# ilyakurdyukov/jpeg-quantsmooth

Measured on AMD Instinct MI355X. Metric: 8x8 blocks/s at q=3 niter=3, higher is better.
Workload: dtype f32

## Files before the change

### include/jpegqs_hip.h

```cpp
#ifndef JPEGQS_HIP_H
#define JPEGQS_HIP_H

#include <stddef.h>
#include <stdint.h>

#ifdef __cplusplus
extern "C" {
#endif

#define QS_HIP_MAXC 4

enum {
	QS_HIP_OK = 0,
	QS_HIP_ENODEV = -1,
	QS_HIP_EINVAL = -2,
	QS_HIP_ENOMEM = -3,
	QS_HIP_ENOTSUP = -4
};


typedef struct {
	int32_t ncomp;
	int32_t colorspace;
	int32_t image_width, image_height;
// ... 234 lines not shown
const char *qs_hip_last_error(void);
#define QS_HIP_ABI_VERSION 7
int qs_hip_abi_version(void);

size_t qs_hip_consts_bytes(void);
size_t qs_hip_plane_pitch(int wblk);
size_t qs_hip_plane_bytes(int wblk, int hblk);
size_t qs_hip_plane_row_offset(int wblk, int y);

int qs_hip_consts_build(void *host_out, const uint16_t quant[64], int flags);

int qs_hip_idct_plane(const void *d_consts, int16_t *d_coef, uint8_t *d_plane,
		int wblk, int hblk, int first, int rep_top, int rep_bot,
		int32_t *d_status, void *stream);

int qs_hip_smooth_plane(const void *d_consts, int16_t *d_coef, const uint8_t *d_plane,
		int wblk, int hblk, int flags, int luma, int final_clamp, void *stream);
int qs_hip_smooth_plane_next(const void *d_consts, int16_t *d_coef, const uint8_t *d_plane, uint8_t *d_plane_next,
		int wblk, int hblk, int flags, int luma, int final_clamp, int rep_top, int rep_bot, void *stream);
int qs_hip_smooth_rows(const void *d_consts, int16_t *d_coef, const uint8_t *d_plane,
		int wblk, int hblk, int row0, int row1, int flags, int luma, int final_clamp, void *stream);

#define QS_HIP_MAX_PLANES 56
typedef struct {
	const void *d_consts;
	int16_t *d_coef;
	uint8_t *d_plane;
	int32_t *d_status;
	int32_t wblk, hblk, luma;
	int32_t band;
} qs_hip_plane_ref;
#define QS_HIP_PLANE_DEFER 4
#define QS_HIP_FIRST_DEFER 2
int qs_hip_idct_planes(const qs_hip_plane_ref *refs, int n, int first, void *stream);
int qs_hip_smooth_planes(const qs_hip_plane_ref *refs, int n, int flags, int final_clamp, void *stream);
int qs_hip_smooth_planes_next(const qs_hip_plane_ref *refs, uint8_t *const *d_plane_next, int n, int flags,
		int final_clamp, void *stream);

int qs_hip_joint_plane(const void *d_consts, int16_t *d_coef, const uint8_t *d_plane,
		const uint8_t *d_luma_lowres, int wblk, int hblk,
		int rebalance, int final_clamp, void *stream);
int qs_hip_lowq_plane(const void *d_consts, int16_t *d_coef, const uint8_t *d_plane,
		int wblk, int hblk, int rebalance, int final_clamp, void *stream);
int qs_hip_downsample_plane(const uint8_t *d_luma, int ywblk, int yhblk, uint8_t *d_lowres,
		int lwblk, int lhblk, int ws, int hs, void *stream);
size_t qs_hip_upsample_pitch(int image_width, int ws);
size_t qs_hip_upsample_bytes(int image_width, int image_height, int ws, int hs);
int qs_hip_upsample_plane(const uint8_t *d_chroma, const uint8_t *d_luma_lowres, int cwblk,
		const uint8_t *d_luma, int ywblk, int yhblk, uint8_t *d_pixels,
		int image_width, int image_height, int ws, int hs, void *stream);
int qs_hip_upsample_rows(const uint8_t *d_chroma, const uint8_t *d_luma_lowres, int cwblk,
		const uint8_t *d_luma, int ywblk, int yhblk, uint8_t *d_pixels, size_t pitch,
		int w1, int h1, int first_rows, int ws, int hs, void *stream);
int qs_hip_fdct_plane(const uint8_t *d_pixels, size_t pitch, int16_t *d_coef, int wblk, int hblk, void *stream);

int qs_hip_clamp_plane(int16_t *d_coef, int wblk, int hblk, void *stream);
int qs_hip_dequant_plane(const void *d_consts, int16_t *d_coef, int wblk, int hblk, void *stream);

#ifdef __cplusplus
}
#endif
#endif
```

### jpeg-quantsmooth_amd/bands.py

```python
from __future__ import annotations

import os
from dataclasses import dataclass


_LIB = None


def _lib():
    global _LIB
    if _LIB is None:
        try:
            from .hipqs import HipQS
            _LIB = HipQS()
        except (OSError, RuntimeError, ImportError):
            _LIB = False
    return _LIB or None


def _band_rows_py(hblk: int, world: int, rank: int, align: int = 1):
    if hblk < 0 or world < 1 or not 0 <= rank < world or align < 1:
        raise ValueError("band_rows: bad argument")
    units = (hblk + align - 1) // align
    a, b = units * rank // world * align, units * (rank + 1) // world * align
# ... 148 lines not shown
        o = offs[y]
        return planes2d[:, o:o + pitch]
    ops, recvs = [], []
    for nbr, src_y, dst_y in ((topo.up, 0, -1), (topo.down, h - 1, h)):
        if nbr is None:
            continue
        out = view(src_y).contiguous()
        if hostcopy:
            out = out.to("cpu")
        buf = out.new_empty(out.shape)
        ops.append(dist.P2POp(dist.isend, out, nbr))
        ops.append(dist.P2POp(dist.irecv, buf, nbr))
        recvs.append((dst_y, buf))
    if ops:
        for w in dist.batch_isend_irecv(ops):
            w.wait()
    for dst_y, buf in recvs:
        view(dst_y).copy_(buf)


def run_bands_batched(engines, topo: BandTopology, niter: int, exchange_many) -> None:
    for it in range(niter):
        for e in engines:
            e.idct(it == 0, topo.rep_top, topo.rep_bot)
        exchange_many()
        for e in engines:
            e.smooth(it == niter - 1)


def defer_bit() -> int:
    return 0 if os.environ.get("QS_BANDS_DEFER", "1") == "0" else 4


def run_bands_batched_sets(hip, engines, topo: BandTopology, niter: int, exchange_many, stream=None, mark=None, fused=True) -> None:
    band = (1 if topo.up is not None else 0) | (2 if topo.down is not None else 0)
    flags = engines[0].flags
    s = stream if stream is not None else engines[0]._s()
    if fused:
        for e in engines:
            e.ensure_plane2()
    for it in range(niter):
        q = defer_bit() if it == 0 else 0
        if it == 0 or not fused:
            refs = hip.plane_refs([(e.cst.data_ptr(), e.coef.data_ptr(), e.plane.data_ptr(), e.status.data_ptr(),
                                    e.wblk, e.hblk, e.luma, band | q) for e in engines])
            hip.idct_planes(refs, it == 0, s)
        exchange_many()
        nxt = fused and it < niter - 1
        refs = hip.plane_refs([(e.cst.data_ptr(), e.coef.data_ptr(), e.plane.data_ptr(), e.status.data_ptr(),
                                e.wblk, e.hblk, e.luma, band | q, e.plane2.data_ptr() if nxt else None) for e in engines])
        if mark:
            mark(0)
        hip.smooth_planes(refs, flags, it == niter - 1, s)
        if mark:
            mark(1)
        if nxt:
            for e in engines:
                e.plane, e.plane2 = e.plane2, e.plane


def run_band_edge_first(hip, e, topo: BandTopology, niter: int, exchange, main, side, torch) -> None:
    if e.hblk < 3:
        return run_bands_batched_sets(hip, [e], topo, niter, exchange, stream=main.cuda_stream)
    e.ensure_plane2()
    band_top = 1 if topo.up is not None else 0
    band_bot = 2 if topo.down is not None else 0
    pitch, wb, hb = e.pitch, e.wblk, e.hblk
    row_bytes = wb * 128

    def views(cur, nxt, q):
        c0, p0 = e.coef.data_ptr(), cur.data_ptr()
        n0 = nxt.data_ptr() if nxt is not None else None
        at = lambda base, r: base + r * 8 * pitch if base is not None else None
        top = (e.cst.data_ptr(), c0, p0, e.status.data_ptr(), wb, 1, e.luma, band_top | 2 | q, n0)
        bot = (e.cst.data_ptr(), c0 + (hb - 1) * row_bytes, at(p0, hb - 1), e.status.data_ptr(), wb, 1, e.luma, 1 | band_bot | q, at(n0, hb - 1))
        mid = (e.cst.data_ptr(), c0 + row_bytes, at(p0, 1), e.status.data_ptr(), wb, hb - 2, e.luma, 3 | q, at(n0, 1))
        return hip.plane_refs([top, bot]), hip.plane_refs([mid])
    ev_main, ev_edge = torch.cuda.Event(), torch.cuda.Event()
    whole = hip.plane_refs([(e.cst.data_ptr(), e.coef.data_ptr(), e.plane.data_ptr(), e.status.data_ptr(), wb, hb, e.luma,
                             band_top | band_bot | (defer_bit() if niter > 0 else 0))])
    hip.idct_planes(whole, True, main.cuda_stream)
    ev_main.record(main)
    side.wait_event(ev_main)
# ... 399 lines not shown
```

### jpeg-quantsmooth_amd/csrc/check_kernel_budget.py

```python
#!/usr/bin/env python3
import re
import sys

KERNELS = ("qs_smooth_plane_kernel", "qs_smooth_set_kernel")
MAX_VGPRS = 168
MAX_LDS = 160 * 1024 // 3
FIELDS = ("group_segment_fixed_size", "private_segment_fixed_size", "vgpr_count")


def kernel_records(text):
    m = re.search(r"^\s*\.amdgpu_metadata\s*$(.*?)^\s*\.end_amdgpu_metadata\s*$", text, re.S | re.M)
    if not m:
        return {}
    recs, cur = [], None
    for line in m.group(1).split("\n"):
        if re.match(r"  - \.", line):
            cur = {}
            recs.append(cur)
            line = "    " + line[4:]
        f = re.match(r"    \.(\w+):\s*(\S+)\s*$", line)
        if f and cur is not None:
            cur[f.group(1)] = f.group(2)
    return {r["name"]: {k: int(r[k]) for k in FIELDS if k in r} for r in recs if "name" in r}


def main(path):
    recs = {n: r for n, r in kernel_records(open(path).read()).items() if any(k in n for k in KERNELS)}
    if len(recs) != 4 or any(len(r) != len(FIELDS) for r in recs.values()):
        print(f"check_kernel_budget: ERROR: expected the metadata of 4 recovery kernels in {path}, found {sorted(recs)}", file=sys.stderr)
        return 1
    bad = 0
    for n, r in sorted(recs.items()):
        why = []
        if r["private_segment_fixed_size"] != 0:
            why.append(f"{r['private_segment_fixed_size']} B of scratch per lane (spills)")
        if r["vgpr_count"] > MAX_VGPRS:
            why.append(f"{r['vgpr_count']} VGPRs > {MAX_VGPRS} (three waves per SIMD)")
        if r["group_segment_fixed_size"] > MAX_LDS:
            why.append(f"{r['group_segment_fixed_size']} B of LDS > {MAX_LDS} (three workgroups per CU)")
        print(f"check_kernel_budget: {n}: {r['vgpr_count']} VGPRs, {r['private_segment_fixed_size']} B scratch, "
              f"{r['group_segment_fixed_size']} B LDS" + (" -- ERROR: " + "; ".join(why) if why else ""),
              file=sys.stderr if why else sys.stdout)
        bad += bool(why)
    return 1 if bad else 0


SPLIT_READ_KERNELS = ("qrs_map", "qrs_decode", "qrs_count", "qrs_tile_scan", "qrs_write", "qrs_dc_tiles", "qrs_dc_write")
DECODE_KERNELS = ("qs_decode_kernel", "qs_decode_scaled_kernel")
PROG_KERNELS = ("qp_begin", "qp_nofile", "qp_flags", "qp_headscan", "qp_runs", "qp_size", "qp_emit", "qp_frame",
                "qr_flags", "qr_wsum", "qr_wscan", "qr_next", "qr_hop")
READ_PROG_KERNELS = ("qrp_init", "qrp_check", "qrp_decode")
INSTANCES = {"qp_size": 4, "qp_emit": 2}


def main_no_scratch(prefix, path):
    want = [k for k in SPLIT_READ_KERNELS + DECODE_KERNELS + PROG_KERNELS + READ_PROG_KERNELS if k.startswith(prefix)]
    recs = kernel_records(open(path).read())
    bad = 0
    for k in want:
        hits = {n: r for n, r in recs.items() if re.search(rf"\d+{k}[EI\d]", n)}
        if len(hits) != INSTANCES.get(k, 1) or any("private_segment_fixed_size" not in r for r in hits.values()):
            count = {1: "one kernel"}.get(INSTANCES.get(k, 1), f"{INSTANCES.get(k, 1)} kernels")
            print(f"check_kernel_budget: ERROR: expected the metadata of {count} {k} in {path}, found {sorted(hits)}", file=sys.stderr)
            bad += 1
            continue
        for n, r in sorted(hits.items()):
            scratch = r["private_segment_fixed_size"]
            print(f"check_kernel_budget: {n}: {r.get('vgpr_count')} VGPRs, {scratch} B scratch, {r.get('group_segment_fixed_size')} B LDS"
                  + (" -- ERROR: scratch" if scratch else ""), file=sys.stderr if scratch else sys.stdout)
            bad += bool(scratch)
    return 1 if bad or not want else 0


if __name__ == "__main__":
    if len(sys.argv) == 4 and sys.argv[1] == "--no-scratch":
        sys.exit(main_no_scratch(sys.argv[2], sys.argv[3]))
    sys.exit(main(sys.argv[1]))
```

### jpeg-quantsmooth_amd/csrc/qs_device.h

```cpp
#pragma once
#include <stdint.h>

#define QS_APRON_X 16
#define QS_LDS_PITCH 65
#define QS_TAB_MAX 272

enum {
  QS_DIAGONALS = 1, QS_JOINT_YUV = 2, QS_UPSAMPLE_UV = 4, QS_LOW_QUALITY = 8,
  QS_NO_REBALANCE = 16, QS_NO_REBALANCE_UV = 32, QS_TRANSCODE = 64
};

struct QsConsts {
  int32_t nat[64];
  int32_t q[64];
  int32_t qraw[64];
  int32_t x1[64];
  int32_t x2[64];
  float   range[64];
  int32_t qn[64], x1n[64], x2n[64];
  int32_t tab_size;
  int32_t pad[15];
  float   tab[64 * QS_TAB_MAX];
  int32_t rec[64][4];
};
enum {
  QS_REC_H_ANY = 1,
  QS_REC_H_SKIP4 = 2,
  QS_REC_H_EVEN = 4,
  QS_REC_V_ANY = 8,
  QS_REC_V_SKIP4 = 16,
  QS_REC_V_EVEN = 32,
  QS_REC_LDS_SHIFT = 6,
  QS_REC_NXT_SHIFT = 12,
  QS_REC_Q1 = 1 << 21
};

static inline int qs_plane_pitch(int wblk) {
  return ((wblk * 8 + QS_APRON_X + 1) + 63) & ~63;
}

#define QS_MAX_PLANES 56
struct QsPlaneRef {
  const QsConsts* cst;
  int16_t* coef;
  uint8_t* plane;
  int32_t* status;
  int32_t wblk, hblk, pitch;
  int32_t mode;
  uint8_t* plane_next;
};
enum {
  QS_PLANE_REBALANCE = 1,
  QS_PLANE_REP_TOP = 2,
  QS_PLANE_REP_BOT = 4,
  QS_PLANE_QUANT = 8
};
struct QsPlaneAux {
  const uint8_t* p[QS_MAX_PLANES];
};
struct QsPlaneSet {
  int32_t n, pad;
  int32_t wave0[QS_MAX_PLANES + 2];
  QsPlaneRef ref[QS_MAX_PLANES];
};
```

### jpeg-quantsmooth_amd/csrc/qs_fused.cpp

```cpp
#include <list>

#include "qs_jobint.h"

using namespace qsx;
using namespace qsj;


namespace {
static size_t plane_stride(int wb, int hb) { return (qs_hip_plane_bytes(wb, hb) + 255) & ~(size_t)255; }
struct FPlane { int job, ci, wb, hb, cst; size_t coef_off, px_off, cbytes; int src_row0, keep0, keep1; };
struct FGroup {
  std::vector<FPlane> planes;
  std::vector<int> jobs;
  DevBuf coef, px, cst, status;
  PinnedBuf stage;
  std::vector<QsConsts> hc;
  PinnedBuf hstatus;
  Download down;
  hipStream_t s = nullptr;
  size_t blocks = 0, coef_bytes = 0;
  std::vector<hipEvent_t> it_ev;
  long long units = 0;
  PinnedBuf hstatus0;
  hipEvent_t ev_status0 = nullptr;
// ... 135 lines not shown
      host_pieces(jobs[P.job], P.ci, P.src_row0, P.hb, P.coef_off, pieces);
    G.coef_bytes = coef_bytes;
    const double t_up0 = wall_ms();
    HIP_TRY(upload_pieces(G.coef.p, pieces, coef_bytes, G.s, G.stage));
    if (trace_on())
      fprintf(stderr, "qs_hip trace: fused  group %zu: alloc+consts %.2f ms, upload of %.1f MiB in %zu piece(s) %.2f ms (%s)\n",
              gi, t_up0 - t_g0, coef_bytes / 1048576.0, pieces.size(), wall_ms() - t_up0, G.stage.p ? "staged" : "direct");
    HIP_TRY(hipMemsetAsync(G.status.p, 0, (size_t)np * sizeof(int32_t), G.s));
    if (trace_on()) {
      for (hipEvent_t& e : G.tev) HIP_TRY(hipEventCreate(&e));
      HIP_TRY(hipEventRecord(G.tev[0], G.s));
    }

    QsPlaneSet set;
    memset(&set, 0, sizeof set);
    set.n = np;
    int w = 0;
    for (int i = 0; i < np; ++i) {
      const FPlane& P = G.planes[i];
      set.wave0[i] = w;
      w += (P.wb * P.hb + 63) / 64;
      QsPlaneRef& R = set.ref[i];
      R.cst = G.cst.as<QsConsts>() + P.cst;
      R.coef = reinterpret_cast<int16_t*>(G.coef.as<char>() + P.coef_off);
      R.plane = G.px.as<uint8_t>() + P.px_off;
      R.status = G.status.as<int32_t>() + i;
      R.wblk = P.wb; R.hblk = P.hb; R.pitch = qs_plane_pitch(P.wb);
      R.mode = QS_PLANE_REP_TOP | QS_PLANE_REP_BOT | (comp_rebalance(jobs[P.job], P.ci, flags) ? QS_PLANE_REBALANCE : 0);
    }
    for (int i = np; i < QS_MAX_PLANES + 2; ++i) set.wave0[i] = w;
    const bool quant = niter > 0;
    if (quant) for (int i = 0; i < np; ++i) set.ref[i].mode |= QS_PLANE_QUANT;
    qs_launch_idct_set(set, 1, G.s);
    if (plan) {
      if (!G.hstatus0.alloc((size_t)np * sizeof(int32_t))) return qs_fail(QS_HIP_ENOMEM, "out of pinned host memory");
      HIP_TRY(hipMemcpyAsync(G.hstatus0.p, G.status.p, (size_t)np * sizeof(int32_t), hipMemcpyDeviceToHost, G.s));
      HIP_TRY(hipEventCreateWithFlags(&G.ev_status0, hipEventDisableTiming));
      HIP_TRY(hipEventRecord(G.ev_status0, G.s));
    }
    for (int it = 0; it < niter; ++it) {
      for (int i = 0; i < np; ++i) {
        uint8_t* a = G.px.as<uint8_t>() + G.planes[i].px_off;
        uint8_t* b = a + plane_stride(G.planes[i].wb, G.planes[i].hb);
        set.ref[i].plane = (it & 1) ? b : a;
        set.ref[i].plane_next = it == niter - 1 ? nullptr : (it & 1) ? a : b;
      }
      qs_launch_smooth_set(set, diag, it == niter - 1, G.s);
      if (it == 0) for (int i = 0; i < np; ++i) set.ref[i].mode &= ~QS_PLANE_QUANT;
      if (plan) {
        hipEvent_t e = nullptr;
        HIP_TRY(hipEventCreateWithFlags(&e, hipEventDisableTiming));
        G.it_ev.push_back(e);
        HIP_TRY(hipEventRecord(e, G.s));
      }
    }
    if (plan) for (const FPlane& P : G.planes) G.units += (long long)(P.keep1 - P.keep0) * jobs[P.job]->vsamp[P.ci];
    HIP_TRY(hipGetLastError());
    if (G.tev[1]) HIP_TRY(hipEventRecord(G.tev[1], G.s));
    if (!G.hstatus.alloc((size_t)np * sizeof(int32_t))) return qs_fail(QS_HIP_ENOMEM, "out of pinned host memory");
    HIP_TRY(hipMemcpyAsync(G.hstatus.p, G.status.p, (size_t)np * sizeof(int32_t), hipMemcpyDeviceToHost, G.s));
    HIP_TRY(G.down.issue(G.coef.p, coef_bytes, G.s, rows_active()));
    if (G.tev[2]) HIP_TRY(hipEventRecord(G.tev[2], G.s));
    if (!G.stage.p) for (int ji : G.jobs) if (split[ji]) defer[ji] = 1;
    return QS_HIP_OK;
  };

// ... 111 lines not shown
```

### jpeg-quantsmooth_amd/csrc/qs_kernels.hip

```cpp
#include <hip/hip_runtime.h>
#include <stdint.h>
#include <stdlib.h>
#include "qs_device.h"
#include "qs_devfn.h"



__device__ __forceinline__ void wave_lds_sync() {
  __builtin_amdgcn_fence(__ATOMIC_RELEASE, "wavefront");
  __builtin_amdgcn_wave_barrier();
  __builtin_amdgcn_fence(__ATOMIC_ACQUIRE, "wavefront");
}

__device__ __forceinline__ uint32_t mulc(uint32_t a, int c) {
  return (uint32_t)__mul24((int)a, c);
}

__device__ __forceinline__ uint32_t lshl13_add(uint32_t x, uint32_t b) {
  uint32_t r;
  asm("v_lshl_add_u32 %0, %1, 13, %2" : "=v"(r) : "v"(x), "v"(b));
  return r;
}

__device__ __forceinline__ void idct8(uint32_t (&v)[8], uint32_t bias) {
// ... 282 lines not shown
#ifndef QS_HOIST_DIAG
#define QS_HOIST_DIAG 32
#endif
#ifndef QS_Q1_SKIP
#define QS_Q1_SKIP 1
#endif
#ifndef QS_STASH
#define QS_STASH 1
#endif
#define QS_X_STASH 0
#define QS_X_EDGE 8
#define QS_X_REB 16
#define QS_X_DWORDS 20
static_assert(QS_WAVES_PER_WG * (32 * QS_LDS_PITCH + QS_X_DWORDS * 64) * 4 <= 160 * 1024 / 3, "LDS budget of three workgroups per CU");
typedef unsigned long long __attribute__((address_space(3))) qs_lds_u64;
__device__ __forceinline__ void qs_lds_add64(qs_lds_u64* p, long long v) {
  __hip_atomic_fetch_add(p, (unsigned long long)v, __ATOMIC_RELAXED, __HIP_MEMORY_SCOPE_WAVEFRONT);
}
__device__ __forceinline__ qs_lds_u64* qs_xreb(const uint32_t* col, const uint32_t* lds, int n) {
  typedef const __attribute__((address_space(3))) uint32_t* lds_ptr;
  uint32_t a = (uint32_t)(uintptr_t)(lds_ptr)col;
  asm volatile("" : "+v"(a));
  const uint32_t b = (uint32_t)(uintptr_t)(lds_ptr)lds;
  return (qs_lds_u64*)(a * 2u - b + (uint32_t)((32 * QS_LDS_PITCH + (QS_X_REB + 2 * n) * 64) * 4));
}

#define QS_SMOOTH_KERNEL_NAME qs_smooth_plane_kernel
#include "qs_smooth_kernel.inc"
#undef QS_SMOOTH_KERNEL_NAME
#define QS_SMOOTH_KERNEL_NAME qs_smooth_set_kernel
#define QS_SMOOTH_SET 1
#include "qs_smooth_kernel.inc"
#undef QS_SMOOTH_KERNEL_NAME
#undef QS_SMOOTH_SET

#define QS_DP_KERNEL_NAME qs_smooth_dp_kernel
#include "qs_smooth_dp_kernel.inc"
#undef QS_DP_KERNEL_NAME
#define QS_DP_KERNEL_NAME qs_smooth_dp_set_kernel
#define QS_DP_SET 1
#include "qs_smooth_dp_kernel.inc"
#undef QS_DP_KERNEL_NAME
#undef QS_DP_SET

__global__ void __launch_bounds__(256)
qs_clamp_kernel(int16_t* __restrict__ coef, size_t nvec) {
  size_t i = (size_t)blockIdx.x * 256 + threadIdx.x;
  const size_t stride = (size_t)gridDim.x * 256;
  uint4* p = reinterpret_cast<uint4*>(coef);
  for (; i < nvec; i += stride) {
    uint4 v = p[i];
    uint32_t d[4] = {v.x, v.y, v.z, v.w};
#pragma unroll
    for (int c = 0; c < 4; ++c) {
      int lo = (int16_t)(d[c] & 0xffff), hi = (int32_t)d[c] >> 16;
      lo = min(max(lo, -1023), 1023); hi = min(max(hi, -1023), 1023);
      d[c] = ((uint32_t)lo & 0xffffu) | ((uint32_t)hi << 16);
    }
    p[i] = make_uint4(d[0], d[1], d[2], d[3]);
  }
}

__global__ void __launch_bounds__(256)
qs_dequant_kernel(const QsConsts* __restrict__ cst, int16_t* __restrict__ coef, size_t nvec) {
  size_t i = (size_t)blockIdx.x * 256 + threadIdx.x;
  const size_t stride = (size_t)gridDim.x * 256;
// ... 40 lines not shown
  if (const int nw = qs_dp_waves((n + 63) / 64)) {
    const dim3 g((n + 63) / 64), b(64 * nw);
#define QS_GO_DP(D, W) hipLaunchKernelGGL((qs_smooth_dp_kernel<D, W>), g, b, 0, s, cst, coef, plane, plane_next, rep, wblk, hblk, pitch, rebalance, final_clamp, blk_begin, blk_end)
    if (nw == 2) { if (diag) QS_GO_DP(true, 2); else QS_GO_DP(false, 2); }
    else if (diag) QS_GO_DP(true, QS_DP_WAVES); else QS_GO_DP(false, QS_DP_WAVES);
#undef QS_GO_DP
    return;
  }
  const int per_wg = 64 * QS_WAVES_PER_WG;
  const dim3 grid((n + per_wg - 1) / per_wg), block(per_wg);
#define QS_GO(K) hipLaunchKernelGGL(K, grid, block, 0, s, cst, coef, plane, plane_next, rep, wblk, hblk, pitch, rebalance, final_clamp, blk_begin, blk_end)
  if (diag) QS_GO(qs_smooth_plane_kernel<true>); else QS_GO(qs_smooth_plane_kernel<false>);
#undef QS_GO
}

void qs_launch_idct_set(const QsPlaneSet& set, int first, hipStream_t s) {
  const int nw = set.wave0[set.n];
  if (nw <= 0) return;
  hipLaunchKernelGGL(qs_idct_set_kernel, dim3((nw + 3) / 4), dim3(256), 0, s, set, first);
}

void qs_launch_smooth_set(const QsPlaneSet& set, int diag, int final_clamp, hipStream_t s) {
  const int nw = set.wave0[set.n];
  if (nw <= 0) return;
  if (const int dw = qs_dp_waves(nw)) {
    const dim3 g(nw), b(64 * dw);
#define QS_GO_DP(D, W) hipLaunchKernelGGL((qs_smooth_dp_set_kernel<D, W>), g, b, 0, s, set, final_clamp)
    if (dw == 2) { if (diag) QS_GO_DP(true, 2); else QS_GO_DP(false, 2); }
    else if (diag) QS_GO_DP(true, QS_DP_WAVES); else QS_GO_DP(false, QS_DP_WAVES);
#undef QS_GO_DP
    return;
  }
  const dim3 grid((nw + QS_WAVES_PER_WG - 1) / QS_WAVES_PER_WG), block(64 * QS_WAVES_PER_WG);
  if (diag) hipLaunchKernelGGL(qs_smooth_set_kernel<true>, grid, block, 0, s, set, final_clamp);
  else      hipLaunchKernelGGL(qs_smooth_set_kernel<false>, grid, block, 0, s, set, final_clamp);
}

void qs_launch_clamp(int16_t* coef, size_t nblk, hipStream_t s) {
  const size_t nvec = nblk * 8;
  const int grid = (int)((nvec + 255) / 256 < 8192 ? (nvec + 255) / 256 : 8192);
  hipLaunchKernelGGL(qs_clamp_kernel, dim3(grid ? grid : 1), dim3(256), 0, s, coef, nvec);
}

void qs_launch_dequant(const QsConsts* cst, int16_t* coef, size_t nblk, hipStream_t s) {
  const size_t nvec = nblk * 8;
  const int grid = (int)((nvec + 255) / 256 < 8192 ? (nvec + 255) / 256 : 8192);
  hipLaunchKernelGGL(qs_dequant_kernel, dim3(grid ? grid : 1), dim3(256), 0, s, cst, coef, nvec);
}
```

### jpeg-quantsmooth_amd/csrc/qs_planes.cpp

```cpp
#include "qs_common.h"


static int check_plane_args(const void* a, const void* b, int wblk, int hblk, const char* who) {
  if (!a || !b) return qs_fail(QS_HIP_EINVAL, "%s: null device pointer", who);
  if (wblk <= 0 || hblk <= 0 || (long long)wblk * hblk > (1ll << 28))
    return qs_fail(QS_HIP_EINVAL, "%s: bad plane size %dx%d blocks", who, wblk, hblk);
  return 0;
}


extern "C" int qs_hip_band_rows(int hblk, int nbands, int band, int align, int* row0, int* row1) {
  if (hblk < 0 || nbands < 1 || band < 0 || band >= nbands || align < 1 || !row0 || !row1)
    return qs_fail(QS_HIP_EINVAL, "qs_hip_band_rows: bad argument");
  const long long units = ((long long)hblk + align - 1) / align;
  const long long a = units * band / nbands * align, b = units * (band + 1) / nbands * align;
  *row0 = (int)(a < hblk ? a : hblk);
  *row1 = (int)(b < hblk ? b : hblk);
  return QS_HIP_OK;
}

extern "C" int qs_hip_colour_band_rows(int hblk_luma, int hblk_chroma, int v_samp, int nbands, int band,
                                       int* y0, int* y1, int* c0, int* c1) {
  if (v_samp < 1 || !y0 || !y1 || !c0 || !c1) return qs_fail(QS_HIP_EINVAL, "qs_hip_colour_band_rows: bad argument");
  if (int r = qs_hip_band_rows(hblk_chroma, nbands, band, 1, c0, c1)) return r;
// ... 52 lines not shown
}

extern "C" int qs_hip_smooth_plane_next(const void* d_consts, int16_t* d_coef, const uint8_t* d_plane, uint8_t* d_plane_next,
                                        int wblk, int hblk, int flags, int luma, int final_clamp, int rep_top, int rep_bot, void* stream) {
  return smooth_rows(d_consts, d_coef, d_plane, wblk, hblk, 0, hblk, flags, luma, final_clamp, stream, "qs_hip_smooth_plane_next",
                     d_plane_next, rep_top, rep_bot);
}

extern "C" int qs_hip_smooth_rows(const void* d_consts, int16_t* d_coef, const uint8_t* d_plane,
                                  int wblk, int hblk, int row0, int row1, int flags, int luma, int final_clamp, void* stream) {
  return smooth_rows(d_consts, d_coef, d_plane, wblk, hblk, row0, row1, flags, luma, final_clamp, stream, "qs_hip_smooth_rows");
}

static int build_plane_set(const qs_hip_plane_ref* refs, uint8_t* const* next, int n, int flags, QsPlaneSet& set, const char* who) {
  if (!refs || n < 1 || n > QS_MAX_PLANES) return qs_fail(QS_HIP_EINVAL, "%s: 1..%d planes per launch", who, QS_MAX_PLANES);
  memset(&set, 0, sizeof set);
  set.n = n;
  int w = 0;
  for (int i = 0; i < n; ++i) {
    const qs_hip_plane_ref& r = refs[i];
    if (int e = check_plane_args(r.d_coef, r.d_plane, r.wblk, r.hblk, who)) return e;
    if (!r.d_consts) return qs_fail(QS_HIP_EINVAL, "%s: null consts", who);
    set.wave0[i] = w;
    w += (r.wblk * r.hblk + 63) / 64;
    QsPlaneRef& R = set.ref[i];
    R.cst = static_cast<const QsConsts*>(r.d_consts);
    R.coef = r.d_coef; R.plane = r.d_plane; R.status = r.d_status;
    R.plane_next = next ? next[i] : nullptr;
    if (R.plane_next && R.plane_next == r.d_plane)
      return qs_fail(QS_HIP_EINVAL, "%s: d_plane_next must be a different buffer (other blocks still read d_plane)", who);
    R.wblk = r.wblk; R.hblk = r.hblk; R.pitch = qs_plane_pitch(r.wblk);
    R.mode = ((!(flags & QS_NO_REBALANCE) && (r.luma || !(flags & QS_NO_REBALANCE_UV))) ? QS_PLANE_REBALANCE : 0) |
             ((r.band & 1) ? 0 : QS_PLANE_REP_TOP) | ((r.band & 2) ? 0 : QS_PLANE_REP_BOT) |
             ((r.band & QS_HIP_PLANE_DEFER) ? QS_PLANE_QUANT : 0);
  }
  for (int i = n; i < QS_MAX_PLANES + 2; ++i) set.wave0[i] = w;
  return QS_HIP_OK;
}

extern "C" int qs_hip_idct_planes(const qs_hip_plane_ref* refs, int n, int first, void* stream) {
  QsPlaneSet set;
  if (int r = build_plane_set(refs, nullptr, n, 0, set, "qs_hip_idct_planes")) return r;
  if (first)
    for (int i = 0; i < n; ++i)
      if (!refs[i].d_status) return qs_fail(QS_HIP_EINVAL, "qs_hip_idct_planes: first pass needs d_status");
  qs_launch_idct_set(set, first, static_cast<hipStream_t>(stream));
  return launch_status("qs_hip_idct_planes");
}

static int smooth_planes(const qs_hip_plane_ref* refs, uint8_t* const* next, int n, int flags, int final_clamp, void* stream, const char* who) {
  if (flags & (QS_JOINT_YUV | QS_UPSAMPLE_UV | QS_LOW_QUALITY))
    return qs_fail(QS_HIP_ENOTSUP, "%s: flags 0x%x need the cross-component stages", who, flags);
  QsPlaneSet set;
  if (int r = build_plane_set(refs, next, n, flags, set, who)) return r;
  qs_launch_smooth_set(set, (flags & QS_DIAGONALS) != 0, final_clamp, static_cast<hipStream_t>(stream));
  return launch_status(who);
}

extern "C" int qs_hip_smooth_planes(const qs_hip_plane_ref* refs, int n, int flags, int final_clamp, void* stream) {
  return smooth_planes(refs, nullptr, n, flags, final_clamp, stream, "qs_hip_smooth_planes");
}

extern "C" int qs_hip_smooth_planes_next(const qs_hip_plane_ref* refs, uint8_t* const* d_plane_next, int n, int flags,
                                         int final_clamp, void* stream) {
  return smooth_planes(refs, d_plane_next, n, flags, final_clamp, stream, "qs_hip_smooth_planes_next");
}

// ... 79 lines not shown
```

### jpeg-quantsmooth_amd/csrc/qs_shard.cpp

```cpp
#include <string>

#include <dlfcn.h>
#include <rccl/rccl.h>

#include "qs_jobint.h"

using namespace qsx;
using namespace qsj;

namespace {

static void band_rows(int hblk, int n, int d, int& r0, int& r1) {
  (void)qs_hip_band_rows(hblk, n, d, 1, &r0, &r1);
}

struct BandPlane {
  int ci = 0, wb = 0, hb = 0, r0 = 0;
  int own0 = 0, own_hb = -1;
  int own_rows() const { return own_hb < 0 ? hb : own_hb; }
  size_t own_off() const { return coef_off + (size_t)own0 * wb * 128; }
  bool halo_top = false, halo_bot = false;
  size_t coef_off = 0, px_off = 0, cbytes = 0;
  int cst = -1;
};
// ... 146 lines not shown
static int stage_band(Band& B, const qs_hip_job* job, int flags) {
  size_t coef_bytes = 0, px_bytes = 0;
  for (BandPlane& P : B.planes) {
    P.cbytes = (size_t)P.wb * P.hb * 128;
    P.coef_off = coef_bytes; coef_bytes += P.cbytes;
    P.px_off = px_bytes; px_bytes += 2 * plane_stride(P.wb, P.hb);
  }
  const int np = (int)B.planes.size();
  HIP_TRY(B.coef.alloc(std::max<size_t>(coef_bytes, 64)));
  HIP_TRY(B.px.alloc(std::max<size_t>(px_bytes, 64)));
  HIP_TRY(B.status.alloc((size_t)std::max(np, 1) * sizeof(int32_t)));
  if (int r = upload_consts(B, job, flags)) return r;
  std::vector<Piece> pieces;
  for (const BandPlane& P : B.planes)
    host_pieces(job, P.ci, P.r0, P.hb, P.coef_off, pieces);
  if (coef_bytes) HIP_TRY(upload_pieces(B.coef.p, pieces, coef_bytes, B.s, B.stage));
  HIP_TRY(hipMemsetAsync(B.status.p, 0, (size_t)std::max(np, 1) * sizeof(int32_t), B.s));

  QsPlaneSet& set = B.set;
  memset(&set, 0, sizeof set);
  set.n = np;
  int w = 0;
  for (int i = 0; i < np; ++i) {
    const BandPlane& P = B.planes[i];
    set.wave0[i] = w;
    w += (P.wb * P.hb + 63) / 64;
    QsPlaneRef& R = set.ref[i];
    R.cst = B.cst.as<QsConsts>() + P.cst;
    R.coef = reinterpret_cast<int16_t*>(B.coef.as<char>() + P.coef_off);
    R.plane = B.px.as<uint8_t>() + P.px_off;
    R.status = B.status.as<int32_t>() + i;
    R.wblk = P.wb; R.hblk = P.hb; R.pitch = qs_plane_pitch(P.wb);
    R.mode = (comp_rebalance(job, P.ci, flags) ? QS_PLANE_REBALANCE : 0) |
             (P.halo_top ? 0 : QS_PLANE_REP_TOP) | (P.halo_bot ? 0 : QS_PLANE_REP_BOT);
  }
  for (int i = np; i < QS_MAX_PLANES + 2; ++i) set.wave0[i] = w;
  return QS_HIP_OK;
}

static const BandPlane* find_plane(const Band& B, int ci) {
  for (const BandPlane& P : B.planes) if (P.ci == ci) return &P;
  return nullptr;
}

static int read_flags(Bands& bands, bool& bad) {
  bad = false;
  for (Band& B : bands.b) {
    HIP_TRY(hipSetDevice(B.dev));
    HIP_TRY(B.down.wait_first(B.s));
    const int32_t* hst = static_cast<const int32_t*>(B.hstatus.p);
    for (size_t i = 0; i < B.planes.size(); ++i) bad |= hst[i] != 0;
  }
  return QS_HIP_OK;
}

static void restore_bands(Bands& bands, const qs_hip_job* job) {
  for (Band& B : bands.b) {
    (void)hipSetDevice(B.dev);
    (void)hipStreamSynchronize(B.s);
    if (!B.stage.p) continue;
    std::vector<Piece> pcs;
    for (const BandPlane& P : B.planes) host_pieces(job, P.ci, P.r0 + P.own0, P.own_rows(), P.own_off(), pcs);
    for (const Piece& pc : pcs) memcpy(pc.host, static_cast<const char*>(B.stage.p) + pc.off, pc.len);
  }
}
#define HIP_TRY_RESTORE(expr) do { hipError_t e_ = (expr); if (e_ != hipSuccess) { restore_bands(bands, job); \
  return qs_fail(e_ == hipErrorOutOfMemory ? QS_HIP_ENOMEM : QS_HIP_ENODEV, "%s failed: %s", #expr, hipGetErrorString(e_)); } } while (0)
// ... 610 lines not shown
```

### jpeg-quantsmooth_amd/csrc/qs_smooth_kernel.inc

```
template <bool DIAG>
__global__ void __launch_bounds__(64 * QS_WAVES_PER_WG, QS_SMOOTH_MIN_WAVES)
#ifdef QS_SMOOTH_SET
QS_SMOOTH_KERNEL_NAME(const QsPlaneSet set, int final_clamp) {
  __shared__ __attribute__((aligned(16))) uint32_t lds_all[QS_WAVES_PER_WG][32 * QS_LDS_PITCH + (DIAG ? 0 : QS_X_DWORDS * 64)];
#if QS_STASH
  __shared__ uint32_t stash_all[QS_WAVES_PER_WG][2 * 8 * 64];
#endif
  const int lane = threadIdx.x & 63, wave = DIAG ? (int)(threadIdx.x >> 6) : __builtin_amdgcn_readfirstlane((int)(threadIdx.x >> 6));
  uint32_t* lds = lds_all[wave];
  uint32_t* col = lds + lane;
  const int gw = __builtin_amdgcn_readfirstlane((int)(blockIdx.x * QS_WAVES_PER_WG + wave));
  if (gw >= set.wave0[set.n]) return;
  const int pi = qs_set_find(set, gw);
  const QsConsts* __restrict__ cst = set.ref[pi].cst;
  int16_t* __restrict__ coef = set.ref[pi].coef;
  const uint8_t* __restrict__ plane = set.ref[pi].plane;
  const int wblk = set.ref[pi].wblk, hblk = set.ref[pi].hblk, pitch = set.ref[pi].pitch;
  const int rebalance = set.ref[pi].mode & QS_PLANE_REBALANCE;
  const int nblk = wblk * hblk;
  const int base = (gw - set.wave0[pi]) * 64;
  (void)hblk;
#else
QS_SMOOTH_KERNEL_NAME(const QsConsts* __restrict__ cst, int16_t* __restrict__ coef,
                       const uint8_t* __restrict__ plane, uint8_t* __restrict__ plane_next, int rep,
// ... 24 lines not shown
  if (set.ref[pi].mode & QS_PLANE_QUANT) {
    const int m0 = (lane & 7) * 4;
    int q[8], unused = 0;
    qs_load_qraw8(cst, lane & 7, q);
#pragma unroll
    for (int j = 0; j < 8; ++j) {
      const int idx = j * 64 + lane;
      uint4 v = make_uint4(0, 0, 0, 0);
      if (idx < nvec) v = gsrc[idx];
      v = qs_dequant8<false>(v, q, unused);
      QS_BIG_ACC(v);
      uint32_t* dst = lds + m0 * QS_LDS_PITCH + (j * 8 + (lane >> 3));
      dst[0] = v.x; dst[QS_LDS_PITCH] = v.y; dst[2 * QS_LDS_PITCH] = v.z; dst[3 * QS_LDS_PITCH] = v.w;
    }
  } else
#endif
  {
    const int m0 = (lane & 7) * 4;
#pragma unroll
    for (int j = 0; j < 8; ++j) {
      const int idx = j * 64 + lane;
      uint4 v = make_uint4(0, 0, 0, 0);
      if (idx < nvec) v = gsrc[idx];
      QS_BIG_ACC(v);
      uint32_t* dst = lds + m0 * QS_LDS_PITCH + (j * 8 + (lane >> 3));
      dst[0] = v.x; dst[QS_LDS_PITCH] = v.y; dst[2 * QS_LDS_PITCH] = v.z; dst[3 * QS_LDS_PITCH] = v.w;
    }
  }

  const int blk = min(base + lane, nblk - 1);
  const int by = blk / wblk, bx = blk - by * wblk;
  const uint8_t* org = plane + (size_t)(by * 8 + 1) * pitch + QS_APRON_X + bx * 8;
  uint32_t edge[8];
  {
    const uint2 t = *reinterpret_cast<const uint2*>(org - pitch);
    const uint2 b = *reinterpret_cast<const uint2*>(org + (size_t)8 * pitch);
    edge[0] = t.x; edge[1] = t.y; edge[2] = b.x; edge[3] = b.y;
    uint32_t l[8], r[8];
#pragma unroll
    for (int y = 0; y < 8; ++y) {
      l[y] = org[(ptrdiff_t)y * pitch - 1];
      r[y] = org[(ptrdiff_t)y * pitch + 8];
    }
    edge[4] = l[0] | (l[1] << 8) | (l[2] << 16) | (l[3] << 24);
    edge[5] = l[4] | (l[5] << 8) | (l[6] << 16) | (l[7] << 24);
    edge[6] = r[0] | (r[1] << 8) | (r[2] << 16) | (r[3] << 24);
    edge[7] = r[4] | (r[5] << 8) | (r[6] << 16) | (r[7] << 24);
  }
  uint32_t* const xcol = col + 32 * QS_LDS_PITCH;
  if constexpr (!DIAG) {
#pragma unroll
    for (int e = 0; e < 8; ++e) xcol[(QS_X_EDGE + e) * 64] = edge[e];
    *qs_xreb(col, lds, 0) = 0; *qs_xreb(col, lds, 1) = 0;
  }
  wave_lds_sync();

  constexpr int TS = DIAG ? 272 : 160;
  float px[DIAG ? 64 : 1];
  float bd[32];
  constexpr int NH = DIAG ? QS_HOIST_DIAG : 1;
  float hd[NH];
  float dh[DIAG ? 1 : 56], dv[DIAG ? 1 : 56];

  int kfirst = 63;
#if QS_STASH
  int stash_hi = 0;
#endif
  uint32_t chg = 0;
  uint64_t chg_any = 0;
#undef QS_BIG_ACC
  const bool big_wave = !DIAG && __builtin_amdgcn_ballot_w64((bigacc & 0xC000C000u) != 0) != 0;
  long long reb_m0 = 0, reb_m1 = 0;
  const float* tabp = cst->tab;
  const int32_t* recp = &cst->rec[0][0];
  qs_w16 WA, WB;
  qs_i4 REC;
  qs_i4 RECN;
  asm volatile("s_load_dwordx4 %0, %2, %3\n\ts_load_dwordx16 %1, %4, %5\n\ts_waitcnt lgkmcnt(0)"
               : "=&s"(REC), "=&s"(WA) : "s"(recp), "s"(63u * 16u), "s"(tabp), "s"((uint32_t)63 * (TS * 4)) : "memory");
  RECN = REC;

#pragma unroll 1
  for (int g = 0; g < 14; ++g) {
    __builtin_amdgcn_s_setprio(QS_PRIO_SLOW);
    if (g == 0 || (DIAG ? __builtin_amdgcn_ballot_w64(chg != 0) != 0 : chg_any != 0)) {
      chg = 0;
      chg_any = 0;
      uint32_t ws[64];
      if constexpr (DIAG) lds_read_block_i16(col, ws); else lds_read_block_i16_1(col, ws);
#if QS_STASH
      {
        uint32_t* stash = DIAG ? stash_all[wave] + lane : xcol + QS_X_STASH * 64;
#pragma unroll
        for (int x = 0; x < 8; ++x) {
          uint32_t c[8];
          const bool low = x <= (DIAG ? 1 : 0), high = x >= (DIAG ? 6 : 7);
          const int slot = (x == 0 || x == 7) ? 0 : 1;
          bool reuse = false, store = false;
          if (low) { reuse = g >= 1 && g <= 7 - x; store = g == 0; }
          if (high) {
            const int fin = 15 - x;
            const bool have = (stash_hi >> (x - 6)) & 1;
            reuse = g >= fin && have; store = g >= fin && !have;
          }
          if ((low || high) && reuse) {
#pragma unroll
            for (int j = 0; j < 8; ++j) c[j] = stash[(slot * 8 + j) * 64];
          } else {
#pragma unroll
            for (int j = 0; j < 8; ++j) c[j] = ws[j * 8 + x];
            idct8(c, 1024u);
#pragma unroll
            for (int j = 0; j < 8; ++j) c[j] = (uint32_t)((int32_t)c[j] >> 11);
            if ((low || high) && store) {
#pragma unroll
              for (int j = 0; j < 8; ++j) stash[(slot * 8 + j) * 64] = c[j];
              if (high) stash_hi |= 1 << (x - 6);
            }
          }
#pragma unroll
          for (int j = 0; j < 8; ++j) ws[j * 8 + x] = c[j];
        }
      }
#else
      idct_pass1(ws);
#endif
      if constexpr (!DIAG) {
        float prev[8];
#pragma unroll
        for (int y = 0; y < 8; ++y) {
          uint32_t row[8]; float o[8];
#pragma unroll
          for (int j = 0; j < 8; ++j) row[j] = ws[y * 8 + j];
          idct_pass2_row_f(row, o);
#pragma unroll
          for (int x = 0; x < 7; ++x) dh[y * 7 + x] = o[x] - o[x + 1];
          if (y > 0) {
#pragma unroll
            for (int x = 0; x < 8; ++x) dv[(y - 1) * 8 + x] = prev[x] - o[x];
          }
          if (y == 0 || y == 7) {
            const uint32_t e0 = xcol[(QS_X_EDGE + (y ? 2 : 0)) * 64], e1 = xcol[(QS_X_EDGE + (y ? 3 : 1)) * 64];
#pragma unroll
            for (int x = 0; x < 8; ++x) bd[(y ? 8 : 0) + x] = o[x] - pix_from_byte(x < 4 ? e0 : e1, x & 3);
          }
          {
            const uint32_t el = xcol[(QS_X_EDGE + 4 + (y >> 2)) * 64], er = xcol[(QS_X_EDGE + 6 + (y >> 2)) * 64];
            bd[16 + y] = o[0] - pix_from_byte(el, y & 3);
            bd[24 + y] = o[7] - pix_from_byte(er, y & 3);
          }
// ... 277 lines not shown
```

### jpeg-quantsmooth_amd/hipqs.py

```python
from __future__ import annotations

import ctypes as C
from pathlib import Path

import numpy as np

PKG_DIR = Path(__file__).resolve().parent
MAXC = 4


class FLAGS:
    DIAGONALS = 1
    JOINT_YUV = 2
    UPSAMPLE_UV = 4
    LOW_QUALITY = 8
    NO_REBALANCE = 16
    NO_REBALANCE_UV = 32
    TRANSCODE = 64
    MASK = 0x7F
    ITER_MAX = 100


def flags_for_quality(quality: int) -> int:
    q = int(quality)
# ... 117 lines not shown
class ReadOpts(C.Structure):
    _fields_ = [("dc", HuffTable * 4), ("ac", HuffTable * 4), ("has_dc", C.c_uint8 * 4), ("has_ac", C.c_uint8 * 4),
                ("dc_tbl", C.c_int32 * MAXC), ("ac_tbl", C.c_int32 * MAXC), ("restart_interval", C.c_int32)]


class ReadInfo(C.Structure):
    _fields_ = [("blocks_in_mcu", C.c_int32), ("mcus", C.c_int32), ("intervals", C.c_int32),
                ("blocks_per_interval", C.c_int64)]


class ReadSplitInfo(C.Structure):
    _fields_ = ReadInfo._fields_ + [("max_segments", C.c_int64)]


class ReadProgScan(C.Structure):
    _fields_ = [("scan", EncodeScan), ("dc_tbl", C.c_int32 * MAXC), ("ac_tbl", C.c_int32 * MAXC), ("dc", HuffTable * 4),
                ("ac", HuffTable * 4), ("has_dc", C.c_uint8 * 4), ("has_ac", C.c_uint8 * 4), ("restart_interval", C.c_int32),
                ("offset", C.c_uint64)]


class ReadProgOpts(C.Structure):
    _fields_ = [("scans", C.POINTER(ReadProgScan)), ("nscans", C.c_int32)]


class ReadProgInfo(C.Structure):
    _fields_ = [("nscans", C.c_int32), ("levels", C.c_int32), ("mcus", C.c_int32 * MAX_SCANS),
                ("intervals", C.c_int32 * MAX_SCANS)]


READ_SPLIT_BYTES = 256
READ_SPLIT_ROUNDS = 17

MAX_PLANES = 56
COMPRESS_CHUNK = 44
DOWNSAMPLE_BOX = 0
DOWNSAMPLE_DCT = 1
DOWNSAMPLING = {"box": DOWNSAMPLE_BOX, "dct": DOWNSAMPLE_DCT}
DECODE_CHUNK = 44
UPSAMPLE_DCT = 0
UPSAMPLE_TRIANGLE = 1
UPSAMPLING = {"dct": UPSAMPLE_DCT, "triangle": UPSAMPLE_TRIANGLE}
PROGRESS_FN = C.CFUNCTYPE(C.c_int, C.c_void_p, C.c_int, C.c_int)

ABI = {
    "qs_hip_do_quantsmooth": (C.c_int, [C.POINTER(Job), C.c_int, C.c_int, C.c_int, PROGRESS_FN, C.c_void_p]),
    "qs_hip_do_quantsmooth_batch": (C.c_int, [C.POINTER(C.POINTER(Job)), C.c_int, C.c_int, C.c_int, C.POINTER(C.c_int)]),
    "qs_hip_do_quantsmooth_rows": (C.c_int, [C.POINTER(Job), C.POINTER(C.POINTER(C.c_void_p)), C.c_int, C.c_int, C.c_int,
                                          PROGRESS_FN, C.c_void_p]),
    "qs_hip_set_devices": (C.c_int, [C.POINTER(C.c_int), C.c_int]),
    "qs_hip_set_shard_schedule": (C.c_int, [C.c_int]),
    "qs_hip_do_quantsmooth_band": (C.c_int, [C.POINTER(Job), C.c_int, C.c_int, C.c_int, C.c_int, C.c_void_p]),
    "qs_hip_do_quantsmooth_sharded": (C.c_int, [C.POINTER(Job), C.c_int, C.c_int, C.POINTER(C.c_int), C.c_int]),
    "qs_hip_band_rows": (C.c_int, [C.c_int, C.c_int, C.c_int, C.c_int, C.POINTER(C.c_int), C.POINTER(C.c_int)]),
    "qs_hip_colour_band_rows": (C.c_int, [C.c_int, C.c_int, C.c_int, C.c_int, C.c_int] + [C.POINTER(C.c_int)] * 4),
    "qs_hip_band_halo_rows": (C.c_int, [C.c_int, C.c_int] + [C.POINTER(C.c_size_t)] * 5),
    "qs_hip_prewarm": (C.c_int, [C.POINTER(Job), C.c_int, C.c_int]),
    "qs_hip_progress_calls": (C.c_int, [C.POINTER(Job), C.c_int, C.c_int, C.POINTER(C.c_int), C.c_int, C.POINTER(C.c_int)]),
    "qs_hip_device_job_info": (C.c_int, [C.POINTER(Job), C.c_int, C.c_int, C.POINTER(DeviceInfo)]),
    "qs_hip_device_job_prepare": (C.c_int, [C.POINTER(Job), C.c_int, C.c_int, C.c_void_p, C.c_size_t, C.c_void_p]),
    "qs_hip_do_quantsmooth_device": (C.c_int, [C.POINTER(Job), C.c_int, C.c_int, C.c_void_p, C.c_size_t, C.c_void_p,
                                               C.c_void_p]),
    "qs_hip_device_batch_info": (C.c_int, [C.POINTER(C.POINTER(Job)), C.c_int, C.c_int, C.c_int, C.POINTER(DeviceInfo),
                                            C.POINTER(C.c_size_t)]),
    "qs_hip_device_batch_prepare": (C.c_int, [C.POINTER(C.POINTER(Job)), C.c_int, C.c_int, C.c_int, C.c_void_p, C.c_size_t,
                                               C.c_void_p]),
    "qs_hip_do_quantsmooth_device_batch": (C.c_int, [C.POINTER(C.POINTER(Job)), C.c_int, C.c_int, C.c_int, C.c_void_p,
# ... 766 lines not shown
```

Baseline: 284.0 million.

## Seed smooth kernel gradients from the existing pixel plane instead of iteration-zero IDCT

Adds a seeded variant of the non-diagonal smooth set kernel. It reads the block's already-reconstructed pixels from the plane and computes the horizontal, vertical and border differences directly, so the first pass no longer has to run an IDCT at g==0. The variant is used whenever every plane in a launch carries the new seeded flag, which the fused, shard and band paths now set by default. In exchange it adds an extra kernel variant, an extra 8-row plane load per block, and changes to the stash reuse logic, which could raise register pressure or alter results if the plane and the coefficients disagree.

Result: no change. 285.2 million, median of 6 (+0.4%).

```diff
diff --git a/include/jpegqs_hip.h b/include/jpegqs_hip.h
--- a/include/jpegqs_hip.h
+++ b/include/jpegqs_hip.h
@@ -290,6 +290,7 @@
 } qs_hip_plane_ref;
 #define QS_HIP_PLANE_DEFER 4
 #define QS_HIP_FIRST_DEFER 2
+#define QS_HIP_PLANE_SEEDED 8
 int qs_hip_idct_planes(const qs_hip_plane_ref *refs, int n, int first, void *stream);
 int qs_hip_smooth_planes(const qs_hip_plane_ref *refs, int n, int flags, int final_clamp, void *stream);
 int qs_hip_smooth_planes_next(const qs_hip_plane_ref *refs, uint8_t *const *d_plane_next, int n, int flags,
diff --git a/jpeg-quantsmooth_amd/bands.py b/jpeg-quantsmooth_amd/bands.py
--- a/jpeg-quantsmooth_amd/bands.py
+++ b/jpeg-quantsmooth_amd/bands.py
@@ -204,6 +204,10 @@
     return 0 if os.environ.get("QS_BANDS_DEFER", "1") == "0" else 4
 
 
+def seed_bit() -> int:
+    return 0 if os.environ.get("QS_BANDS_SEED", "1") == "0" else 8
+
+
 def run_bands_batched_sets(hip, engines, topo: BandTopology, niter: int, exchange_many, stream=None, mark=None, fused=True) -> None:
     band = (1 if topo.up is not None else 0) | (2 if topo.down is not None else 0)
     flags = engines[0].flags
@@ -219,8 +223,9 @@
             hip.idct_planes(refs, it == 0, s)
         exchange_many()
         nxt = fused and it < niter - 1
+        sd = seed_bit()
         refs = hip.plane_refs([(e.cst.data_ptr(), e.coef.data_ptr(), e.plane.data_ptr(), e.status.data_ptr(),
-                                e.wblk, e.hblk, e.luma, band | q, e.plane2.data_ptr() if nxt else None) for e in engines])
+                                e.wblk, e.hblk, e.luma, band | q | sd, e.plane2.data_ptr() if nxt else None) for e in engines])
         if mark:
             mark(0)
         hip.smooth_planes(refs, flags, it == niter - 1, s)
diff --git a/jpeg-quantsmooth_amd/csrc/check_kernel_budget.py b/jpeg-quantsmooth_amd/csrc/check_kernel_budget.py
--- a/jpeg-quantsmooth_amd/csrc/check_kernel_budget.py
+++ b/jpeg-quantsmooth_amd/csrc/check_kernel_budget.py
@@ -3,6 +3,7 @@
 import sys
 
 KERNELS = ("qs_smooth_plane_kernel", "qs_smooth_set_kernel")
+SEEDED = "qs_smooth_seeded_kernel"
 MAX_VGPRS = 168
 MAX_LDS = 160 * 1024 // 3
 FIELDS = ("group_segment_fixed_size", "private_segment_fixed_size", "vgpr_count")
@@ -24,11 +25,17 @@
     return {r["name"]: {k: int(r[k]) for k in FIELDS if k in r} for r in recs if "name" in r}
 
 
-def main(path):
-    recs = {n: r for n, r in kernel_records(open(path).read()).items() if any(k in n for k in KERNELS)}
+def main(path, seeded=False):
+    every = kernel_records(open(path).read())
+    recs = {n: r for n, r in every.items() if any(k in n for k in KERNELS)}
     if len(recs) != 4 or any(len(r) != len(FIELDS) for r in recs.values()):
         print(f"check_kernel_budget: ERROR: expected the metadata of 4 recovery kernels in {path}, found {sorted(recs)}", file=sys.stderr)
         return 1
+    more = {n: r for n, r in every.items() if SEEDED in n}
+    if seeded and (len(more) != 1 or any(len(r) != len(FIELDS) for r in more.values())):
+        print(f"check_kernel_budget: ERROR: expected the metadata of one {SEEDED} in {path}, found {sorted(more)}", file=sys.stderr)
+        return 1
+    recs.update(more)
     bad = 0
     for n, r in sorted(recs.items()):
         why = []
@@ -75,4 +82,6 @@
 if __name__ == "__main__":
     if len(sys.argv) == 4 and sys.argv[1] == "--no-scratch":
         sys.exit(main_no_scratch(sys.argv[2], sys.argv[3]))
+    if len(sys.argv) == 3 and sys.argv[1] == "--seeded":
+        sys.exit(main(sys.argv[2], seeded=True))
     sys.exit(main(sys.argv[1]))
diff --git a/jpeg-quantsmooth_amd/csrc/qs_device.h b/jpeg-quantsmooth_amd/csrc/qs_device.h
--- a/jpeg-quantsmooth_amd/csrc/qs_device.h
+++ b/jpeg-quantsmooth_amd/csrc/qs_device.h
@@ -53,7 +53,8 @@
   QS_PLANE_REBALANCE = 1,
   QS_PLANE_REP_TOP = 2,
   QS_PLANE_REP_BOT = 4,
-  QS_PLANE_QUANT = 8
+  QS_PLANE_QUANT = 8,
+  QS_PLANE_SEEDED = 16
 };
 struct QsPlaneAux {
   const uint8_t* p[QS_MAX_PLANES];
diff --git a/jpeg-quantsmooth_amd/csrc/qs_fused.cpp b/jpeg-quantsmooth_amd/csrc/qs_fused.cpp
--- a/jpeg-quantsmooth_amd/csrc/qs_fused.cpp
+++ b/jpeg-quantsmooth_amd/csrc/qs_fused.cpp
@@ -191,6 +191,7 @@
     const bool quant = niter > 0;
     if (quant) for (int i = 0; i < np; ++i) set.ref[i].mode |= QS_PLANE_QUANT;
     qs_launch_idct_set(set, 1, G.s);
+    for (int i = 0; i < np; ++i) set.ref[i].mode |= QS_PLANE_SEEDED;
     if (plan) {
       if (!G.hstatus0.alloc((size_t)np * sizeof(int32_t))) return qs_fail(QS_HIP_ENOMEM, "out of pinned host memory");
       HIP_TRY(hipMemcpyAsync(G.hstatus0.p, G.status.p, (size_t)np * sizeof(int32_t), hipMemcpyDeviceToHost, G.s));
diff --git a/jpeg-quantsmooth_amd/csrc/qs_kernels.hip b/jpeg-quantsmooth_amd/csrc/qs_kernels.hip
--- a/jpeg-quantsmooth_amd/csrc/qs_kernels.hip
+++ b/jpeg-quantsmooth_amd/csrc/qs_kernels.hip
@@ -338,6 +338,11 @@
 #define QS_SMOOTH_SET 1
 #include "qs_smooth_kernel.inc"
 #undef QS_SMOOTH_KERNEL_NAME
+#define QS_SMOOTH_KERNEL_NAME qs_smooth_seeded_kernel
+#define QS_SMOOTH_SEEDED 1
+#include "qs_smooth_kernel.inc"
+#undef QS_SMOOTH_KERNEL_NAME
+#undef QS_SMOOTH_SEEDED
 #undef QS_SMOOTH_SET
 
 #define QS_DP_KERNEL_NAME qs_smooth_dp_kernel
@@ -444,7 +449,10 @@
     return;
   }
   const dim3 grid((nw + QS_WAVES_PER_WG - 1) / QS_WAVES_PER_WG), block(64 * QS_WAVES_PER_WG);
+  bool seeded = !diag;
+  for (int i = 0; i < set.n; ++i) seeded = seeded && (set.ref[i].mode & QS_PLANE_SEEDED);
   if (diag) hipLaunchKernelGGL(qs_smooth_set_kernel<true>, grid, block, 0, s, set, final_clamp);
+  else if (seeded) hipLaunchKernelGGL(qs_smooth_seeded_kernel<false>, grid, block, 0, s, set, final_clamp);
   else      hipLaunchKernelGGL(qs_smooth_set_kernel<false>, grid, block, 0, s, set, final_clamp);
 }
 
diff --git a/jpeg-quantsmooth_amd/csrc/qs_planes.cpp b/jpeg-quantsmooth_amd/csrc/qs_planes.cpp
--- a/jpeg-quantsmooth_amd/csrc/qs_planes.cpp
+++ b/jpeg-quantsmooth_amd/csrc/qs_planes.cpp
@@ -108,7 +108,8 @@
     R.wblk = r.wblk; R.hblk = r.hblk; R.pitch = qs_plane_pitch(r.wblk);
     R.mode = ((!(flags & QS_NO_REBALANCE) && (r.luma || !(flags & QS_NO_REBALANCE_UV))) ? QS_PLANE_REBALANCE : 0) |
              ((r.band & 1) ? 0 : QS_PLANE_REP_TOP) | ((r.band & 2) ? 0 : QS_PLANE_REP_BOT) |
-             ((r.band & QS_HIP_PLANE_DEFER) ? QS_PLANE_QUANT : 0);
+             ((r.band & QS_HIP_PLANE_DEFER) ? QS_PLANE_QUANT : 0) |
+             ((r.band & QS_HIP_PLANE_SEEDED) ? QS_PLANE_SEEDED : 0);
   }
   for (int i = n; i < QS_MAX_PLANES + 2; ++i) set.wave0[i] = w;
   return QS_HIP_OK;
diff --git a/jpeg-quantsmooth_amd/csrc/qs_shard.cpp b/jpeg-quantsmooth_amd/csrc/qs_shard.cpp
--- a/jpeg-quantsmooth_amd/csrc/qs_shard.cpp
+++ b/jpeg-quantsmooth_amd/csrc/qs_shard.cpp
@@ -202,7 +202,7 @@
     R.status = B.status.as<int32_t>() + i;
     R.wblk = P.wb; R.hblk = P.hb; R.pitch = qs_plane_pitch(P.wb);
     R.mode = (comp_rebalance(job, P.ci, flags) ? QS_PLANE_REBALANCE : 0) |
-             (P.halo_top ? 0 : QS_PLANE_REP_TOP) | (P.halo_bot ? 0 : QS_PLANE_REP_BOT);
+             (P.halo_top ? 0 : QS_PLANE_REP_TOP) | (P.halo_bot ? 0 : QS_PLANE_REP_BOT) | QS_PLANE_SEEDED;
   }
   for (int i = np; i < QS_MAX_PLANES + 2; ++i) set.wave0[i] = w;
   return QS_HIP_OK;
diff --git a/jpeg-quantsmooth_amd/csrc/qs_smooth_kernel.inc b/jpeg-quantsmooth_amd/csrc/qs_smooth_kernel.inc
--- a/jpeg-quantsmooth_amd/csrc/qs_smooth_kernel.inc
+++ b/jpeg-quantsmooth_amd/csrc/qs_smooth_kernel.inc
@@ -80,6 +80,18 @@
   const int by = blk / wblk, bx = blk - by * wblk;
   const uint8_t* org = plane + (size_t)(by * 8 + 1) * pitch + QS_APRON_X + bx * 8;
   uint32_t edge[8];
+#ifdef QS_SMOOTH_SEEDED
+  constexpr bool seeded = !DIAG;
+#else
+  constexpr bool seeded = false;
+#endif
+  uint2 own[8];
+  if constexpr (!DIAG) {
+    if (seeded) {
+#pragma unroll
+      for (int y = 0; y < 8; ++y) own[y] = *reinterpret_cast<const uint2*>(org + (ptrdiff_t)y * pitch);
+    }
+  }
   {
     const uint2 t = *reinterpret_cast<const uint2*>(org - pitch);
     const uint2 b = *reinterpret_cast<const uint2*>(org + (size_t)8 * pitch);
@@ -128,10 +140,46 @@
                : "=&s"(REC), "=&s"(WA) : "s"(recp), "s"(63u * 16u), "s"(tabp), "s"((uint32_t)63 * (TS * 4)) : "memory");
   RECN = REC;
 
+  if constexpr (!DIAG) {
+    if (seeded) {
+      __builtin_amdgcn_s_setprio(QS_PRIO_SLOW);
+      float prev[8];
+#pragma unroll
+      for (int y = 0; y < 8; ++y) {
+        float o[8];
+#pragma unroll
+        for (int x = 0; x < 8; ++x) o[x] = pix_from_byte(x < 4 ? own[y].x : own[y].y, x & 3);
+#pragma unroll
+        for (int x = 0; x < 7; ++x) dh[y * 7 + x] = o[x] - o[x + 1];
+        if (y > 0) {
+#pragma unroll
+          for (int x = 0; x < 8; ++x) dv[(y - 1) * 8 + x] = prev[x] - o[x];
+        }
+        if (y == 0 || y == 7) {
+          const uint32_t e0 = xcol[(QS_X_EDGE + (y ? 2 : 0)) * 64], e1 = xcol[(QS_X_EDGE + (y ? 3 : 1)) * 64];
+#pragma unroll
+          for (int x = 0; x < 8; ++x) bd[(y ? 8 : 0) + x] = o[x] - pix_from_byte(x < 4 ? e0 : e1, x & 3);
+        }
+        {
+          const uint32_t el = xcol[(QS_X_EDGE + 4 + (y >> 2)) * 64], er = xcol[(QS_X_EDGE + 6 + (y >> 2)) * 64];
+          bd[16 + y] = o[0] - pix_from_byte(el, y & 3);
+          bd[24 + y] = o[7] - pix_from_byte(er, y & 3);
+        }
+#pragma unroll
+        for (int x = 0; x < 8; ++x) prev[x] = o[x];
+        __builtin_amdgcn_sched_barrier(0);
+      }
+    }
+  }
+
 #pragma unroll 1
   for (int g = 0; g < 14; ++g) {
     __builtin_amdgcn_s_setprio(QS_PRIO_SLOW);
+#ifdef QS_SMOOTH_SEEDED
+    if (DIAG ? __builtin_amdgcn_ballot_w64(chg != 0) != 0 : chg_any != 0) {
+#else
     if (g == 0 || (DIAG ? __builtin_amdgcn_ballot_w64(chg != 0) != 0 : chg_any != 0)) {
+#endif
       chg = 0;
       chg_any = 0;
       uint32_t ws[64];
@@ -145,7 +193,16 @@
           const bool low = x <= (DIAG ? 1 : 0), high = x >= (DIAG ? 6 : 7);
           const int slot = (x == 0 || x == 7) ? 0 : 1;
           bool reuse = false, store = false;
-          if (low) { reuse = g >= 1 && g <= 7 - x; store = g == 0; }
+          if (low) {
+#ifndef QS_SMOOTH_SEEDED
+            reuse = g >= 1 && g <= 7 - x; store = g == 0;
+#else
+            {
+              const bool have = (stash_hi >> 2) & 1;
+              reuse = g <= 7 - x && have; store = g <= 7 - x && !have;
+            }
+#endif
+          }
           if (high) {
             const int fin = 15 - x;
             const bool have = (stash_hi >> (x - 6)) & 1;
@@ -164,6 +221,9 @@
 #pragma unroll
               for (int j = 0; j < 8; ++j) stash[(slot * 8 + j) * 64] = c[j];
               if (high) stash_hi |= 1 << (x - 6);
+#ifdef QS_SMOOTH_SEEDED
+              else stash_hi |= 4;
+#endif
             }
           }
 #pragma unroll
diff --git a/jpeg-quantsmooth_amd/hipqs.py b/jpeg-quantsmooth_amd/hipqs.py
--- a/jpeg-quantsmooth_amd/hipqs.py
+++ b/jpeg-quantsmooth_amd/hipqs.py
@@ -173,6 +173,8 @@
 READ_SPLIT_ROUNDS = 17
 
 MAX_PLANES = 56
+PLANE_DEFER = 4
+PLANE_SEEDED = 8
 COMPRESS_CHUNK = 44
 DOWNSAMPLE_BOX = 0
 DOWNSAMPLE_DCT = 1
```
